# thu-ml/tianshou

Measured on AMD Instinct MI355X. Metric: PPO learn() update-steps/sec (minibatch 65536, preprocessing incl.) + GAE transitions/sec; cpu_baseline / rocm_eager_baseline are PORTS of the reference path (oracle/), kind=port, higher is better.
Workload: dtype f32; 1 GPU; C2 PPO MuJoCo-shape rollout (BASELINE configs[1]): ONE rollout of 512 envs x 2048 steps = 2^20 transitions, minibatch 65536, obs 17, act 6, MLP[64,64] actor-critic, repeat 10, recompute_advantage off; parallelism=dp1, exchange=none

## Files before the change

include/tsengine.h:

```cpp
#ifndef TSENGINE_H
#define TSENGINE_H

#include <stddef.h>
#include <stdint.h>

#ifdef __cplusplus
extern "C" {
#endif

#define TS_OK 0
#define TS_ERR_INVALID_ARG (-1)
#define TS_ERR_SHAPE (-2)
#define TS_ERR_HIP (-3)
#define TS_ERR_UNSUPPORTED (-4)
#define TS_ERR_WORKSPACE (-5)

typedef void* ts_stream_t;
typedef struct ts_workspace ts_workspace;

const char* ts_version(void);
const char* ts_last_error(void);

int ts_workspace_create(ts_workspace** out, int device, size_t max_bytes);
int ts_workspace_destroy(ts_workspace* ws);

int ts_workspace_side_stream(ts_workspace* ws, int which, ts_stream_t* stream_out);

#define TS_KIND_PPO_STEP 0
#define TS_KIND_PPO_REDUCE 1
#define TS_KIND_PPO_ADAM 2
#define TS_KIND_PPO_INFER 3
#define TS_KIND_GAE_MAPS 4
#define TS_KIND_GAE_APPLY 5
#define TS_KIND_CONV_FWD 6
#define TS_KIND_CONV_WGRAD 7
#define TS_KIND_CONV_DGRAD 8
#define TS_N_KINDS 9
int ts_profile_begin(ts_workspace* ws);
int ts_profile_end(ts_workspace* ws, double* h_ms_by_kind, int64_t* h_count_by_kind, int n_kinds);


int64_t ts_gae_num_tiles(int64_t n);
int ts_gae_scan(ts_workspace* ws, const float* v_s, const float* v_s_next, const void* rew,
                int rew_dtype, const uint8_t* terminated, const uint8_t* truncated,
                const int64_t* cut_pos, int64_t n_cut, const int64_t* d_n_cut, int64_t n,
                double gamma, double gae_lambda, double v_scale, double ret_div, float* adv_out,
                float* returns_out, double* adv64, double* ret64, double* ret_partials,
                ts_stream_t stream);

int ts_gae_check(ts_workspace* ws, int* h_error_out, ts_stream_t stream);

int ts_isin_positions(const int64_t* indices, int64_t n, const int64_t* unfinished,
                      int64_t n_unfinished, int64_t* cut_pos_out, int64_t capacity,
                      int64_t* n_cut_out, ts_stream_t stream);

int ts_nstep_return(const double* rew_B, const uint8_t* end_flag_B, const float* target_q_IA,
                    const int64_t* stacked_indices_NI, int64_t I, int64_t A, int64_t n_step,
                    int64_t B, double gamma, float* out, double* out64, ts_stream_t stream);

int ts_nstep_indices(const int64_t* indices, int64_t I, int64_t n_step, const int64_t* offset,
                     int64_t E, const uint8_t* done, const int64_t* last_index,
                     const int64_t* lengths, int64_t* after_out, int64_t* stacked_out,
                     ts_stream_t stream);

int ts_nstep_return_fused(const int64_t* indices, int64_t I, int64_t n_step,
                          const int64_t* offset, int64_t E, const uint8_t* done,
                          const uint8_t* terminated, const int64_t* last_index,
                          const int64_t* lengths, const double* rew_B, const float* target_q_IA,
                          int64_t A, double gamma, float* out, double* out64,
                          ts_stream_t stream);

int ts_nstep_coefficients(const int64_t* indices, int64_t I, int64_t n_step, const int64_t* offset, int64_t E,
                          const uint8_t* done_B, const uint8_t* terminated_B, const int64_t* last_index,
                          const int64_t* lengths, const double* rew_B, double gamma, float* mask_out, double* gpow_out,
                          double* mc_out, ts_stream_t stream);


int ts_next_index(const int64_t* index, int64_t I, const int64_t* offset, int64_t E,
                  const uint8_t* done, const int64_t* last_index, const int64_t* lengths,
                  int64_t* out, ts_stream_t stream);
int ts_prev_index(const int64_t* index, int64_t I, const int64_t* offset, int64_t E,
                  const uint8_t* done, const int64_t* last_index, const int64_t* lengths,
                  int64_t* out, ts_stream_t stream);

int ts_unfinished_index(const int64_t* offset, int64_t E, const uint8_t* done,
                        const int64_t* last_index, const int64_t* lengths, int64_t* out,
                        int64_t* n_out, ts_stream_t stream);

int ts_sample_indices_all(ts_workspace* ws, const int64_t* offset, int64_t E,
                          const int64_t* lengths, const int64_t* insertion, int64_t total,
                          int64_t* out, ts_stream_t stream);

int ts_sample_indices_random(const int64_t* offset, int64_t E, const int64_t* lengths, const double* u_buffer,
                             const int64_t* within_i, const double* within_u, int64_t batch_size, int64_t* out,
                             int* err_flag, ts_stream_t stream);
int ts_sample_indices_seeded(const int64_t* offset, int64_t E, const int64_t* lengths, uint64_t seed, uint64_t counter,
                             int64_t batch_size, int64_t* out, int* err_flag, ts_stream_t stream);

int ts_random_permutation(int64_t* out, int64_t n, uint64_t seed, ts_stream_t stream);

int ts_normal_fill(float* out, int64_t n, uint64_t seed, uint64_t offset, ts_stream_t stream);
// ... 728 lines not shown
```

tianshou_amd/csrc/ts_returns.hip:

```cpp
#include <algorithm>
#include <cstdlib>

#include "ts_common.h"

#pragma clang fp contract(off)

namespace {

constexpr int GAE_THREADS = 256;
constexpr int GAE_ITEMS = 8;
constexpr int GAE_TILE = GAE_THREADS * GAE_ITEMS;
constexpr int GAE_WAVES = GAE_THREADS / 64;

struct Aff {
    double a, b;
};

__device__ __forceinline__ Aff aff_identity() { return Aff{1.0, 0.0}; }

__device__ __forceinline__ Aff compose(const Aff& L, const Aff& R) {
    return Aff{L.a * R.a, L.b + L.a * R.b};
}

__device__ __forceinline__ Aff shfl_down_aff(const Aff& v, int off) {
    return Aff{__shfl_down(v.a, off, 64), __shfl_down(v.b, off, 64)};
}

__device__ __forceinline__ Aff wave_reduce_aff(Aff v, int lane) {
#pragma unroll
    for (int off = 1; off < 64; off <<= 1) {
        Aff r = shfl_down_aff(v, off);
        if (lane + off < 64) v = compose(v, r);
    }
    return v;
}

__device__ __forceinline__ Aff wave_suffix_scan_aff(Aff v, int lane) {
#pragma unroll
    for (int off = 1; off < 64; off <<= 1) {
        Aff r = shfl_down_aff(v, off);
        if (lane + off < 64) v = compose(v, r);
    }
    return v;
}

__device__ __forceinline__ Aff block_reduce_aff(Aff v, Aff* lds ) {
    const int lane = threadIdx.x & 63, wave = threadIdx.x >> 6;
    Aff w = wave_reduce_aff(v, lane);
    __syncthreads();
    if (lane == 0) lds[wave] = w;
    __syncthreads();
    Aff t = lds[0];
#pragma unroll
    for (int k = 1; k < GAE_WAVES; ++k) t = compose(t, lds[k]);
    return t;
}

template <typename RewT>
struct GaeArgs {
    const float* v_s;
    const float* v_n;
    const RewT* rew;
    const uint8_t* term;
    const uint8_t* trunc;
    const int64_t* cut_pos;
    const int64_t* d_n_cut;
    int64_t n_cut;
    int64_t n;
    double gamma, gl, v_scale, ret_div;
    const uint32_t* cutbits;
};

struct GaeRaw {
    float fv[GAE_ITEMS], fn[GAE_ITEMS];
    double rw[GAE_ITEMS];
    uint8_t te[GAE_ITEMS], tr[GAE_ITEMS];
};

template <typename RewT, bool VEC>
__device__ __forceinline__ void gae_load_raw(const GaeArgs<RewT>& g, int64_t base, GaeRaw& r) {
    const bool full = base + GAE_ITEMS <= g.n;
    if (VEC && full) {
        const float4* pv = reinterpret_cast<const float4*>(g.v_s + base);
        const float4* pn = reinterpret_cast<const float4*>(g.v_n + base);
        float4 a0 = pv[0], a1 = pv[1], b0 = pn[0], b1 = pn[1];
        r.fv[0] = a0.x; r.fv[1] = a0.y; r.fv[2] = a0.z; r.fv[3] = a0.w;
        r.fv[4] = a1.x; r.fv[5] = a1.y; r.fv[6] = a1.z; r.fv[7] = a1.w;
        r.fn[0] = b0.x; r.fn[1] = b0.y; r.fn[2] = b0.z; r.fn[3] = b0.w;
        r.fn[4] = b1.x; r.fn[5] = b1.y; r.fn[6] = b1.z; r.fn[7] = b1.w;
        if constexpr (sizeof(RewT) == 4) {
            const float4* pr = reinterpret_cast<const float4*>(g.rew + base);
            float4 r0 = pr[0], r1 = pr[1];
            r.rw[0] = r0.x; r.rw[1] = r0.y; r.rw[2] = r0.z; r.rw[3] = r0.w;
            r.rw[4] = r1.x; r.rw[5] = r1.y; r.rw[6] = r1.z; r.rw[7] = r1.w;
        } else {
            const double2* pr = reinterpret_cast<const double2*>(g.rew + base);
#pragma unroll
            for (int k = 0; k < GAE_ITEMS / 2; ++k) {
                double2 q = pr[k];
                r.rw[2 * k] = q.x;
                r.rw[2 * k + 1] = q.y;
            }
        }
        const uint2 t8 = *reinterpret_cast<const uint2*>(g.term + base);
        const uint2 u8 = *reinterpret_cast<const uint2*>(g.trunc + base);
#pragma unroll
        for (int k = 0; k < 4; ++k) {
            r.te[k] = (t8.x >> (8 * k)) & 0xFF;
            r.te[4 + k] = (t8.y >> (8 * k)) & 0xFF;
            r.tr[k] = (u8.x >> (8 * k)) & 0xFF;
            r.tr[4 + k] = (u8.y >> (8 * k)) & 0xFF;
        }
    } else {
#pragma unroll
        for (int k = 0; k < GAE_ITEMS; ++k) {
            const int64_t i = base + k;
            const bool ok = i < g.n;
            r.fv[k] = ok ? g.v_s[i] : 0.f;
            r.fn[k] = ok ? g.v_n[i] : 0.f;
            r.rw[k] = ok ? (double)g.rew[i] : 0.0;
            r.te[k] = ok ? g.term[i] : (uint8_t)1;
            r.tr[k] = ok ? g.trunc[i] : (uint8_t)1;
// ... 125 lines not shown
            if (base + k < g.n) {
                if (adv64) adv64[base + k] = adv[k];
                if (ret64) ret64[base + k] = ret[k];
            }
    }
}

__device__ __forceinline__ void gae_store_partials(double s1, double s2, int lane, int wave, int64_t tile,
                                                   double* red, double* ret_partials) {
#pragma unroll
    for (int off = 32; off > 0; off >>= 1) {
        s1 += __shfl_down(s1, off, 64);
        s2 += __shfl_down(s2, off, 64);
    }
    if (lane == 0) {
        red[2 * wave] = s1;
        red[2 * wave + 1] = s2;
    }
    __syncthreads();
    if (threadIdx.x == 0) {
        double t1 = 0.0, t2 = 0.0;
        for (int w = 0; w < GAE_WAVES; ++w) {
            t1 += red[2 * w];
            t2 += red[2 * w + 1];
        }
        ret_partials[2 * tile] = t1;
        ret_partials[2 * tile + 1] = t2;
    }
}

constexpr int GAE_SHARDS = 8;

struct GaeSyncHeader {
    struct alignas(128) { unsigned long long v; } ticket[GAE_SHARDS];
    unsigned int error;
    unsigned int pad[3];
};

struct GaeLaunch {
    unsigned long long base[GAE_SHARDS];
    int direct;
};

struct GaeTileMsg {
    unsigned long long a_bits, b_bits;
    unsigned int flag;
    unsigned int pad;
};

constexpr unsigned GAE_SPIN_LIMIT = 1u << 22;


template <typename RewT, bool VEC>
__global__ __launch_bounds__(GAE_THREADS) void gae_single_pass(GaeArgs<RewT> g, GaeSyncHeader* hdr,
                                                               GaeTileMsg* msg, int64_t n_tiles,
                                                               GaeLaunch launch,
                                                               unsigned int epoch, float* adv_out,
                                                               float* ret_out, double* adv64,
                                                               double* ret64, double* ret_partials) {
    __shared__ uint32_t cutmask[GAE_TILE / 32];
    __shared__ Aff lds[GAE_WAVES];
    __shared__ double red[2 * GAE_WAVES];
    __shared__ int64_t tile_s;
    __shared__ int closed_s;
    const int lane = threadIdx.x & 63, wave = threadIdx.x >> 6;
    int64_t tile;
    if (launch.direct) {
        tile = n_tiles - 1 - (int64_t)blockIdx.x;
    } else {
        if (threadIdx.x == 0) {
            const int shard = blockIdx.x & (GAE_SHARDS - 1);
            const unsigned long long t = __hip_atomic_fetch_add(&hdr->ticket[shard].v, 1ULL, __ATOMIC_RELAXED,
                                                                __HIP_MEMORY_SCOPE_AGENT);
            const int64_t seq = (int64_t)(t - launch.base[shard]) * GAE_SHARDS + shard;
            tile_s = n_tiles - 1 - seq;
        }
        __syncthreads();
        tile = tile_s;
    }
    const int64_t tile_start = tile * GAE_TILE;
    double vs[GAE_ITEMS], d[GAE_ITEMS], c[GAE_ITEMS];
    const int64_t base = tile_start + (int64_t)threadIdx.x * GAE_ITEMS;
    {
        GaeRaw raw;
        if (g.cutbits) {
            const GaeCutPre cuts = gae_cut_prefetch(g, tile_start);
            gae_load_raw<RewT, VEC>(g, base, raw);
            gae_cutmask_from_prefetch(g, tile_start, cuts, cutmask);
        } else {
            gae_load_raw<RewT, VEC>(g, base, raw);
            gae_build_cutmask(g, tile_start, cutmask);
        }
        gae_convert(g, base, raw, cutmask, vs, d, c);
    }
    const Aff mine = items_to_aff(d, c);

    const Aff incl = wave_suffix_scan_aff(mine, lane);
    Aff excl = shfl_down_aff(incl, 1);
    if (lane == 63) excl = aff_identity();
    if (lane == 0) lds[wave] = incl;
    if (threadIdx.x == GAE_THREADS - 1) closed_s = c[GAE_ITEMS - 1] == 0.0 ? 1 : 0;
    __syncthreads();
    const bool closed = closed_s != 0;
    Aff wmap[GAE_WAVES];
#pragma unroll
    for (int w = 0; w < GAE_WAVES; ++w) wmap[w] = lds[w];
    if (threadIdx.x == 0) {
        Aff t = wmap[0];
#pragma unroll
        for (int w = 1; w < GAE_WAVES; ++w) t = compose(t, wmap[w]);
        __hip_atomic_store(&msg[tile].a_bits, (unsigned long long)__double_as_longlong(t.a), __ATOMIC_RELAXED,
                           __HIP_MEMORY_SCOPE_AGENT);
        __hip_atomic_store(&msg[tile].b_bits, (unsigned long long)__double_as_longlong(t.b), __ATOMIC_RELAXED,
                           __HIP_MEMORY_SCOPE_AGENT);
        asm volatile("s_waitcnt vmcnt(0)" ::: "memory");
        __hip_atomic_store(&msg[tile].flag, epoch, __ATOMIC_RELAXED, __HIP_MEMORY_SCOPE_AGENT);
    }

    Aff acc = aff_identity();
    int64_t t0 = tile + 1;
    for (int round = 0; !closed && t0 < n_tiles; ++round) {
        const int width = round == 0 ? 1 : (round == 1 ? 15 : (round == 2 ? 240 : GAE_THREADS));
        Aff f = aff_identity();
        const int64_t t = t0 + threadIdx.x;
        if ((int)threadIdx.x < width && t < n_tiles) {
            unsigned spins = 0;
            while (__hip_atomic_load(&msg[t].flag, __ATOMIC_RELAXED, __HIP_MEMORY_SCOPE_AGENT) != epoch) {
                __builtin_amdgcn_s_sleep(1);
                if (++spins > GAE_SPIN_LIMIT) { hdr->error = 1u; break; }
            }
            const unsigned long long ab = __hip_atomic_load(&msg[t].a_bits, __ATOMIC_RELAXED, __HIP_MEMORY_SCOPE_AGENT);
            const unsigned long long bb = __hip_atomic_load(&msg[t].b_bits, __ATOMIC_RELAXED, __HIP_MEMORY_SCOPE_AGENT);
            f = Aff{__longlong_as_double((long long)ab), __longlong_as_double((long long)bb)};
        }
        acc = compose(acc, block_reduce_aff(f, lds));
        if (acc.a == 0.0) break;
        t0 += width;
    }
    double wave_carry = acc.b;
#pragma unroll
    for (int w = GAE_WAVES - 1; w >= 0; --w)
        if (w > wave) wave_carry = wmap[w].b + wmap[w].a * wave_carry;
    double x = excl.b + excl.a * wave_carry;

    double adv[GAE_ITEMS], ret[GAE_ITEMS];
    double s1 = 0.0, s2 = 0.0;
#pragma unroll
    for (int k = GAE_ITEMS - 1; k >= 0; --k) {
        x = d[k] + c[k] * x;
        adv[k] = x;
        ret[k] = x + vs[k];
        if (base + k < g.n) {
            s1 += ret[k];
            s2 += ret[k] * ret[k];
        }
    }
    gae_store_outputs<VEC>(g, base, adv, ret, adv_out, ret_out, adv64, ret64);
    if (ret_partials) gae_store_partials(s1, s2, lane, wave, tile, red, ret_partials);
}

__global__ void isin_positions_kernel(const int64_t* indices, int64_t n, const int64_t* unf,
                                      int64_t n_unf, int64_t* out, int64_t capacity,
                                      unsigned long long* count) {
    const int64_t stride = (int64_t)gridDim.x * blockDim.x;
    for (int64_t i = (int64_t)blockIdx.x * blockDim.x + threadIdx.x; i < n; i += stride) {
        const int64_t v = indices[i];
        int64_t lo = 0, hi = n_unf;
        while (lo < hi) {
            const int64_t mid = (lo + hi) >> 1;
            if (unf[mid] < v) lo = mid + 1; else hi = mid;
        }
        if (lo < n_unf && unf[lo] == v) {
            const unsigned long long p = atomicAdd(count, 1ULL);
            if ((int64_t)p < capacity) out[p] = i;
        }
    }
}

__device__ __forceinline__ int64_t pymod(int64_t a, int64_t m) {
    const int64_t r = a % m;
    return r < 0 ? r + m : r;
}

__device__ __forceinline__ int64_t find_sub(const int64_t* offset, int64_t E, int64_t idx) {
    int64_t lo = 0, hi = E;
    while (hi - lo > 1) {
        const int64_t mid = (lo + hi) >> 1;
        if (offset[mid] <= idx) lo = mid; else hi = mid;
    }
    return lo;
}

__device__ __forceinline__ int64_t next_one(int64_t idx, const int64_t* offset, int64_t E,
                                            const uint8_t* done, const int64_t* last_index,
                                            const int64_t* lengths, bool* is_end) {
    idx = pymod(idx, offset[E]);
    const int64_t e = find_sub(offset, E, idx);
    const int64_t start = offset[e];
    const int64_t len = lengths[e];
    const int64_t cur_len = len > 1 ? len : 1;
    const int64_t end_flag = (done[idx] != 0) | (idx == last_index[e]);
    if (is_end) *is_end = (done[idx] != 0) | (len > 0 && idx == last_index[e]);
    return pymod(idx - start + 1 - end_flag, cur_len) + start;
}

__global__ void nstep_return_kernel(const double* rew, const uint8_t* end_flag, const float* tq,
                                    const int64_t* stacked, int64_t I, int64_t A, int64_t N,
                                    double gamma, float* out, double* out64) {
    const int64_t total = I * A;
    const int64_t stride = (int64_t)gridDim.x * blockDim.x;
    for (int64_t t = (int64_t)blockIdx.x * blockDim.x + threadIdx.x; t < total; t += stride) {
// ... 155 lines not shown
int launch_gae(ts_workspace* ws, const GaeArgs<RewT>& g_in, float* adv_out, float* ret_out,
               double* adv64, double* ret64, double* ret_partials, hipStream_t stream) {
    GaeArgs<RewT> g = g_in;
    const int64_t n_tiles = ts::ceil_div(g.n, GAE_TILE);
    g.cutbits = nullptr;
    if (g.n_cut > GAE_CUT_SCAN_MAX) {
        const size_t words = (size_t)ts::ceil_div(g.n, 32);
        if (int rc = ts::ws_reserve(ws, 4 * words)) return rc;
        uint32_t* bits = reinterpret_cast<uint32_t*>(ws->base);
        TS_HIP_CHECK(hipMemsetAsync(bits, 0, 4 * words, stream));
        const unsigned blocks = (unsigned)std::min<int64_t>(ts::ceil_div(g.n_cut, 256), 1024);
        hipLaunchKernelGGL(gae_cutbits_kernel, dim3(blocks), dim3(256), 0, stream, g.cut_pos, g.n_cut, g.d_n_cut, g.n, bits);
        TS_LAUNCH_CHECK();
        g.cutbits = bits;
    }
    const bool vec = aligned16(g.v_s) && aligned16(g.v_n) && aligned16(g.rew) &&
                     (reinterpret_cast<uintptr_t>(g.term) & 7u) == 0 &&
                     (reinterpret_cast<uintptr_t>(g.trunc) & 7u) == 0 && aligned16(adv_out) &&
                     aligned16(ret_out);
    {
        int rc = gae_sync_reserve(ws, n_tiles, stream);
        if (rc != TS_OK) return rc;
        GaeSyncHeader* hdr = reinterpret_cast<GaeSyncHeader*>(ws->gae_sync);
        GaeTileMsg* msg = reinterpret_cast<GaeTileMsg*>(hdr + 1);
        const unsigned int epoch = ++ws->gae_epoch;
        GaeLaunch base;
        static const int64_t direct_max = getenv("TS_GAE_DIRECT_MAX") ? atoll(getenv("TS_GAE_DIRECT_MAX")) : 1024;
        base.direct = n_tiles <= direct_max ? 1 : 0;
        for (int k = 0; k < GAE_SHARDS; ++k) {
            base.base[k] = ws->gae_ticket_base[k];
            if (!base.direct)
                ws->gae_ticket_base[k] += (unsigned long long)((n_tiles - k + GAE_SHARDS - 1) / GAE_SHARDS);
        }
        ts::ProfScope prof(ws, TS_KIND_GAE_APPLY, stream);
        if (vec)
            hipLaunchKernelGGL((gae_single_pass<RewT, true>), dim3((unsigned)n_tiles), dim3(GAE_THREADS), 0,
                               stream, g, hdr, msg, n_tiles, base, epoch, adv_out, ret_out, adv64, ret64,
                               ret_partials);
        else
            hipLaunchKernelGGL((gae_single_pass<RewT, false>), dim3((unsigned)n_tiles), dim3(GAE_THREADS), 0,
                               stream, g, hdr, msg, n_tiles, base, epoch, adv_out, ret_out, adv64, ret64,
                               ret_partials);
        TS_LAUNCH_CHECK();
        return TS_OK;
    }
}

}

extern "C" {

int64_t ts_gae_num_tiles(int64_t n) { return n <= 0 ? 0 : ts::ceil_div(n, GAE_TILE); }

int ts_gae_scan(ts_workspace* ws, const float* v_s, const float* v_s_next, const void* rew,
                int rew_dtype, const uint8_t* terminated, const uint8_t* truncated,
                const int64_t* cut_pos, int64_t n_cut, const int64_t* d_n_cut, int64_t n,
                double gamma, double gae_lambda, double v_scale, double ret_div, float* adv_out,
                float* returns_out, double* adv64, double* ret64, double* ret_partials,
                ts_stream_t stream) {
    TS_REQUIRE(n >= 0 && n_cut >= 0, TS_ERR_INVALID_ARG, "ts_gae_scan: negative size");
    if (n == 0) return TS_OK;
    TS_REQUIRE(v_s && v_s_next && rew && terminated && truncated && adv_out && returns_out,
               TS_ERR_INVALID_ARG, "ts_gae_scan: NULL array argument");
    TS_REQUIRE(n_cut == 0 || cut_pos, TS_ERR_INVALID_ARG, "ts_gae_scan: cut_pos is NULL");
    TS_REQUIRE(rew_dtype == 0 || rew_dtype == 1, TS_ERR_INVALID_ARG,
               "ts_gae_scan: rew_dtype must be 0 (f32) or 1 (f64)");
    TS_REQUIRE(ret_div != 0.0, TS_ERR_INVALID_ARG, "ts_gae_scan: ret_div must be non-zero");
    hipStream_t s = ts::as_stream(stream);
    if (rew_dtype == 0) {
        GaeArgs<float> g{v_s, v_s_next, (const float*)rew, terminated, truncated, cut_pos, d_n_cut,
                         n_cut, n, gamma, gamma * gae_lambda, v_scale, ret_div};
        return launch_gae(ws, g, adv_out, returns_out, adv64, ret64, ret_partials, s);
    }
    GaeArgs<double> g{v_s, v_s_next, (const double*)rew, terminated, truncated, cut_pos, d_n_cut,
                      n_cut, n, gamma, gamma * gae_lambda, v_scale, ret_div};
    return launch_gae(ws, g, adv_out, returns_out, adv64, ret64, ret_partials, s);
}

int ts_gae_check(ts_workspace* ws, int* error_out, ts_stream_t stream) {
    TS_REQUIRE(ws && error_out, TS_ERR_INVALID_ARG, "ts_gae_check: NULL argument");
    *error_out = 0;
    if (!ws->gae_sync) return TS_OK;
    GaeSyncHeader h;
    hipStream_t s = ts::as_stream(stream);
    TS_HIP_CHECK(hipMemcpyAsync(&h, ws->gae_sync, sizeof(h), hipMemcpyDeviceToHost, s));
    TS_HIP_CHECK(hipStreamSynchronize(s));
    *error_out = (int)h.error;
    return TS_OK;
}

int ts_isin_positions(const int64_t* indices, int64_t n, const int64_t* unfinished,
                      int64_t n_unfinished, int64_t* cut_pos_out, int64_t capacity,
                      int64_t* n_cut_out, ts_stream_t stream) {
    TS_REQUIRE(n >= 0 && n_unfinished >= 0 && capacity >= 0, TS_ERR_INVALID_ARG,
               "ts_isin_positions: negative size");
    TS_REQUIRE(n_cut_out, TS_ERR_INVALID_ARG, "ts_isin_positions: n_cut_out is NULL");
    hipStream_t s = ts::as_stream(stream);
    TS_HIP_CHECK(hipMemsetAsync(n_cut_out, 0, sizeof(int64_t), s));
    if (n == 0 || n_unfinished == 0) return TS_OK;
    TS_REQUIRE(indices && unfinished && cut_pos_out, TS_ERR_INVALID_ARG,
               "ts_isin_positions: NULL array argument");
    hipLaunchKernelGGL(isin_positions_kernel, dim3(grid_for(n, 256)), dim3(256), 0, s, indices, n,
                       unfinished, n_unfinished, cut_pos_out, capacity,
                       reinterpret_cast<unsigned long long*>(n_cut_out));
    TS_LAUNCH_CHECK();
    return TS_OK;
}

int ts_nstep_return(const double* rew_B, const uint8_t* end_flag_B, const float* target_q_IA,
                    const int64_t* stacked_indices_NI, int64_t I, int64_t A, int64_t n_step,
                    int64_t B, double gamma, float* out, double* out64, ts_stream_t stream) {
    TS_REQUIRE(I >= 0 && A >= 0 && B >= 0, TS_ERR_INVALID_ARG, "ts_nstep_return: negative size");
    TS_REQUIRE(n_step >= 1, TS_ERR_INVALID_ARG, "ts_nstep_return: n_step must be >= 1");
    if (I * A == 0) return TS_OK;
    TS_REQUIRE(rew_B && end_flag_B && target_q_IA && stacked_indices_NI && out, TS_ERR_INVALID_ARG,
               "ts_nstep_return: NULL array argument");
    hipLaunchKernelGGL(nstep_return_kernel, dim3(grid_for(I * A, 256)), dim3(256), 0,
                       ts::as_stream(stream), rew_B, end_flag_B, target_q_IA, stacked_indices_NI, I,
                       A, n_step, gamma, out, out64);
    TS_LAUNCH_CHECK();
    return TS_OK;
}

int ts_nstep_indices(const int64_t* indices, int64_t I, int64_t n_step, const int64_t* offset,
                     int64_t E, const uint8_t* done, const int64_t* last_index,
                     const int64_t* lengths, int64_t* after_out, int64_t* stacked_out,
                     ts_stream_t stream) {
    TS_REQUIRE(I >= 0 && E >= 1, TS_ERR_INVALID_ARG, "ts_nstep_indices: bad size");
    TS_REQUIRE(n_step >= 1, TS_ERR_INVALID_ARG, "ts_nstep_indices: n_step must be >= 1");
// ... 50 lines not shown
```

tianshou_amd/ppo.py:

```python
from __future__ import annotations

import ctypes as C
import math
from dataclasses import dataclass

import numpy as np
import torch

from . import _lib
from .buffer import _dev_index
from .returns import gae_scan

HIDDEN = 64
PARAM_ORDER = ("a_w1", "a_b1", "a_w2", "a_b2", "a_wmu", "a_bmu", "a_sigma",
               "c_w1", "c_b1", "c_w2", "c_b2", "c_wv", "c_bv")


def param_shapes(obs_dim: int, act_dim: int) -> dict[str, tuple[int, ...]]:
    return {
        "a_w1": (HIDDEN, obs_dim), "a_b1": (HIDDEN,), "a_w2": (HIDDEN, HIDDEN), "a_b2": (HIDDEN,),
        "a_wmu": (act_dim, HIDDEN), "a_bmu": (act_dim,), "a_sigma": (act_dim,),
        "c_w1": (HIDDEN, obs_dim), "c_b1": (HIDDEN,), "c_w2": (HIDDEN, HIDDEN), "c_b2": (HIDDEN,),
        "c_wv": (1, HIDDEN), "c_bv": (1,),
    }


def param_count(obs_dim: int, act_dim: int) -> int:
    return int(_lib.load().ts_ppo_param_count(_lib.i64(obs_dim), _lib.i64(act_dim)))


TIANSHOU_ACTOR_KEYS = ("preprocess.model.model.0.weight", "preprocess.model.model.0.bias",
                       "preprocess.model.model.2.weight", "preprocess.model.model.2.bias",
                       "mu.model.0.weight", "mu.model.0.bias", "sigma_param")
TIANSHOU_CRITIC_KEYS = ("preprocess.model.model.0.weight", "preprocess.model.model.0.bias",
                        "preprocess.model.model.2.weight", "preprocess.model.model.2.bias",
                        "last.model.0.weight", "last.model.0.bias")


def flat_from_modules(actor, critic, device="cuda") -> torch.Tensor:
    sa, sc = actor.state_dict(), critic.state_dict()
    parts = [sa[k] for k in TIANSHOU_ACTOR_KEYS] + [sc[k] for k in TIANSHOU_CRITIC_KEYS]
    return torch.cat([p.detach().reshape(-1).to(torch.float32) for p in parts]).to(device).contiguous()


def flat_to_modules(flat: torch.Tensor, actor, critic) -> None:
    off = 0
    with torch.no_grad():
        for mod, keys in ((actor, TIANSHOU_ACTOR_KEYS), (critic, TIANSHOU_CRITIC_KEYS)):
            sd = dict(mod.named_parameters())
            for k in keys:
                p = sd[k]
                n = p.numel()
                p.copy_(flat[off:off + n].reshape(p.shape).to(p.device))
                off += n
    assert off == flat.numel()


@dataclass
class PPOConfig:
    algo: str = "ppo"
    gamma: float = 0.99
    gae_lambda: float = 0.95
    eps_clip: float = 0.2
    dual_clip: float | None = None
# ... 69 lines not shown
    ws = _lib.default_workspace(_dev_index(params))
    _lib.check(_lib.load().ts_ppo_infer_bounded(
        ws.handle, _lib.ptr(params), _lib.i64(obs_dim), _lib.i64(act_dim), _lib.f64(max_action or 0.0), _lib.ptr(obs),
        _lib.ptr(act), _lib.i64(n), _lib.ptr(v), _lib.ptr(lp), None, _lib.current_stream(dev)))
    return v, lp


def policy_forward(params: torch.Tensor, obs_dim: int, act_dim: int, obs: torch.Tensor, noise=None, *,
                   bound_method: str | None = "clip", low=None, high=None, max_action: float | None = None,
                   want_mu: bool = False):
    n, dev = obs.shape[0], obs.device
    obs = obs.to(torch.float32).contiguous()
    noise = None if noise is None else torch.as_tensor(noise, device=dev).to(torch.float32).reshape(n, act_dim).contiguous()
    f = lambda x: None if x is None else torch.as_tensor(x, dtype=torch.float32, device=dev).reshape(act_dim).contiguous()
    low, high = f(low), f(high)
    act = torch.empty((n, act_dim), dtype=torch.float32, device=dev)
    mapped = torch.empty_like(act)
    mu = torch.empty_like(act) if want_mu else None
    ws = _lib.default_workspace(_dev_index(params))
    _lib.check(_lib.load().ts_ppo_policy_forward_bounded(
        ws.handle, _lib.ptr(params), _lib.i64(obs_dim), _lib.i64(act_dim), _lib.f64(max_action or 0.0), _lib.ptr(obs),
        _lib.ptr(noise), _lib.i64(n), C.c_int({None: 0, "clip": 1, "tanh": 2}[bound_method]), _lib.ptr(low), _lib.ptr(high),
        _lib.ptr(act), _lib.ptr(mapped), _lib.ptr(mu), _lib.current_stream(dev)))
    return (act, mapped, mu) if want_mu else (act, mapped)


def pack_batch(b: dict, obs_dim: int, act_dim: int) -> torch.Tensor:
    n = b["obs"].shape[0]
    lib = _lib.load()
    lib.ts_ppo_record_width.restype = C.c_int64
    w = int(lib.ts_ppo_record_width(_lib.i64(obs_dim), _lib.i64(act_dim)))
    rec = torch.empty((n, w), dtype=torch.float32, device=b["obs"].device)
    _lib.check(lib.ts_ppo_pack_batch(
        _lib.ptr(b["obs"]), _lib.ptr(b["act"]), _lib.ptr(b["adv"]), _lib.ptr(b["returns"]),
        _lib.ptr(b["logp_old"]), _lib.ptr(b["v_s"]), _lib.i64(n), _lib.i64(obs_dim), _lib.i64(act_dim),
        _lib.ptr(rec), _lib.current_stream(rec.device)))
    return rec


class PPOEngine:

    def __init__(self, obs_dim: int, act_dim: int, flat_params: torch.Tensor, cfg: PPOConfig):
        if not flat_params.is_cuda:
            raise RuntimeError("PPOEngine needs its parameters on an MI355X; there is no CPU fallback")
        self.obs_dim, self.act_dim, self.cfg = obs_dim, act_dim, cfg
        self.P = param_count(obs_dim, act_dim)
        if flat_params.numel() != self.P:
            raise ValueError(f"flat_params has {flat_params.numel()} entries, layout needs {self.P}")
        self.params = flat_params.detach().to(torch.float32).contiguous().clone()
        self.adam_m = torch.zeros_like(self.params)
        self.adam_v = torch.zeros_like(self.params)
        self.adam_step = 0
        self.device = self.params.device
        self.ret_rms = [0.0, 1.0, 0.0]
        self._eps = 1e-8
        self._ws = _lib.default_workspace(_dev_index(self.params))

    def check(self) -> None:
        if self._ws.gae_check():
            raise _lib.EngineError(-1, "gae_single_pass: a tile hand-off timed out; advantages / returns are invalid")

    def _f32(self, x) -> torch.Tensor:
        if not isinstance(x, torch.Tensor):
            x = torch.as_tensor(np.asarray(x), device=self.device)
        return x.to(device=self.device, dtype=torch.float32).contiguous()

    def add_returns_and_advantages(self, obs, obs_next, rew, terminated, truncated, cut_pos,
                                   d_n_cut=None, reduce_stats=None, v_s=None):
        cfg = self.cfg
        if v_s is None:
            v_s, _ = infer(self.params, self.obs_dim, self.act_dim, obs)
        v_next, _ = infer(self.params, self.obs_dim, self.act_dim, obs_next)
        scale = math.sqrt(self.ret_rms[1] + self._eps) if cfg.return_scaling else 1.0
        out = gae_scan(v_s, v_next, rew, terminated, truncated, cut_pos, gamma=cfg.gamma,
                       gae_lambda=cfg.gae_lambda, v_scale=scale, ret_div=scale,
                       want_ret_stats=cfg.return_scaling, d_n_cut=d_n_cut, ws=self._ws)
        if cfg.return_scaling:
            n = float(v_s.numel())
            s1, s2 = float(out["ret_sum"]), float(out["ret_sumsq"])
            if reduce_stats is not None:
                s1, s2, n = reduce_stats(s1, s2, n)
            self.ret_rms = rms_merge(self.ret_rms, s1, s2, n)
        return v_s, out["returns"], out["adv"]

    def preprocess(self, obs, obs_next, act, rew, terminated, truncated, cut_pos, d_n_cut=None, reduce_stats=None):
        obs, obs_next, act = self._f32(obs), self._f32(obs_next), self._f32(act)
        if self.cfg.algo == "a2c":
            v_s, returns, adv = self.add_returns_and_advantages(obs, obs_next, rew, terminated,
                                                                truncated, cut_pos, d_n_cut, reduce_stats)
            logp_old = torch.zeros_like(adv)
        else:
            v_s0, logp_old = infer(self.params, self.obs_dim, self.act_dim, obs, act, want_v=True, want_logp=True,
                                   max_action=self.cfg.max_action)
            v_s, returns, adv = self.add_returns_and_advantages(obs, obs_next, rew, terminated, truncated, cut_pos,
                                                                d_n_cut, reduce_stats, v_s=v_s0)
        return {"obs": obs, "obs_next": obs_next, "act": act, "rew": rew, "terminated": terminated,
                "truncated": truncated, "cut_pos": cut_pos, "d_n_cut": d_n_cut,
                "v_s": v_s, "returns": returns, "adv": adv, "logp_old": logp_old}

    def _run_steps(self, b: dict, perm: torch.Tensor | None, offsets: list[int], want_grad=False):
        n_steps = len(offsets) - 1
        losses = torch.empty((n_steps, 4), dtype=torch.float32, device=self.device)
        grads = torch.empty(self.P, dtype=torch.float32, device=self.device) if want_grad else None
        h_off = (C.c_int64 * len(offsets))(*offsets)
        hp = self.cfg.to_c()
        _lib.check(_lib.load().ts_ppo_update(
            self._ws.handle, _lib.ptr(self.params), _lib.ptr(self.adam_m), _lib.ptr(self.adam_v),
            _lib.i64(self.adam_step), _lib.i64(self.obs_dim), _lib.i64(self.act_dim),
            _lib.ptr(b["obs"]), _lib.ptr(b["act"]), _lib.ptr(b["adv"]), _lib.ptr(b["returns"]),
            _lib.ptr(b["logp_old"]), _lib.ptr(b["v_s"]), _lib.i64(b["obs"].shape[0]), _lib.ptr(perm),
            h_off, _lib.i64(n_steps), C.byref(hp), _lib.ptr(losses), _lib.ptr(grads),
            _lib.current_stream(self.device)))
        self.adam_step += n_steps
        return losses, grads

    def update(self, b: dict, batch_size: int | None, repeat: int, perms=None, want_grad=False):
        n = b["obs"].shape[0]
        cfg = self.cfg
        if perms is None:
            perms = [np.random.permutation(n) for _ in range(repeat)]
        offs1 = split_offsets(n, batch_size, merge_last=True)
        out, grads = [], None
        if not cfg.recompute_advantage:
            if all(isinstance(p, torch.Tensor) for p in perms):
                perm = torch.cat([p.to(device=self.device, dtype=torch.int64) for p in perms])
            else:
                perm = torch.as_tensor(np.concatenate([np.asarray(p, dtype=np.int64) for p in perms]),
                                       device=self.device)
            offsets = [r * n + o for r in range(repeat) for o in offs1[:-1]] + [repeat * n]
            losses, grads = self._run_steps(b, perm, offsets, want_grad)
            out.append(losses)
        else:
            for r in range(repeat):
                if r > 0:
                    v_s, returns, adv = self.add_returns_and_advantages(
# ... 17 lines not shown
```

tianshou_amd/returns.py:

```python
from __future__ import annotations

import numpy as np
import torch

from . import _lib
from .buffer import DeviceReplayBuffer, _dev_index, _i64_dev, _u8_dev


def _f32(x, device) -> torch.Tensor:
    if isinstance(x, torch.Tensor):
        return x.to(device=device, dtype=torch.float32).reshape(-1).contiguous()
    return torch.as_tensor(np.asarray(x, dtype=np.float32).reshape(-1), device=device)


def gae_scan(v_s, v_s_next, rew, terminated, truncated, cut_pos=None, *, gamma=0.99,
             gae_lambda=0.95, v_scale=1.0, ret_div=1.0, want_f64=False, want_ret_stats=False,
             d_n_cut=None, ws=None):
    dev = v_s.device
    v_s = _f32(v_s, dev)
    v_s_next = _f32(v_s_next, dev)
    n = v_s.numel()
    if isinstance(rew, torch.Tensor):
        rew = rew.to(dev).reshape(-1)
        if rew.dtype not in (torch.float32, torch.float64):
            rew = rew.to(torch.float64)
        rew = rew.contiguous()
    else:
        rew = torch.as_tensor(np.asarray(rew, dtype=np.float64).reshape(-1), device=dev)
    terminated, truncated = _u8_dev(terminated, dev).reshape(-1), _u8_dev(truncated, dev).reshape(-1)
    if not (v_s_next.numel() == rew.numel() == terminated.numel() == truncated.numel() == n):
        raise ValueError("gae_scan: input length mismatch")
    n_cut = 0
    if cut_pos is not None:
        cut_pos = _i64_dev(cut_pos, dev).reshape(-1)
        n_cut = cut_pos.numel()
    adv = torch.empty(n, dtype=torch.float32, device=dev)
    ret = torch.empty(n, dtype=torch.float32, device=dev)
    adv64 = torch.empty(n, dtype=torch.float64, device=dev) if want_f64 else None
    ret64 = torch.empty(n, dtype=torch.float64, device=dev) if want_f64 else None
    lib = _lib.load()
    parts = None
    if want_ret_stats:
        parts = torch.zeros(2 * max(int(lib.ts_gae_num_tiles(n)), 1), dtype=torch.float64, device=dev)
    if ws is None:
        ws = _lib.default_workspace(_dev_index(v_s))
    _lib.check(lib.ts_gae_scan(
        ws.handle, _lib.ptr(v_s), _lib.ptr(v_s_next), _lib.ptr(rew),
        0 if rew.dtype == torch.float32 else 1, _lib.ptr(terminated), _lib.ptr(truncated),
        _lib.ptr(cut_pos), _lib.i64(n_cut), _lib.ptr(d_n_cut), _lib.i64(n), _lib.f64(gamma),
        _lib.f64(gae_lambda), _lib.f64(v_scale), _lib.f64(ret_div), _lib.ptr(adv), _lib.ptr(ret),
        _lib.ptr(adv64), _lib.ptr(ret64), _lib.ptr(parts), _lib.current_stream(dev)))
    out = {"adv": adv, "returns": ret}
    if want_f64:
        out["adv64"], out["ret64"] = adv64, ret64
    if want_ret_stats:
        p = parts.view(-1, 2).sum(dim=0)
        out["ret_sum"], out["ret_sumsq"] = p[0], p[1]
    return out


def _gae(v_s, v_s_, rew, end_flag, gamma: float, gae_lambda: float) -> torch.Tensor:
    dev = v_s.device if isinstance(v_s, torch.Tensor) else torch.device("cuda")
    end = _u8_dev(end_flag, dev)
    zeros = torch.zeros_like(end)
    return gae_scan(_f32(v_s, dev), _f32(v_s_, dev), rew, zeros, end, gamma=gamma,
                    gae_lambda=gae_lambda, want_f64=True)["adv64"]


def cut_positions(buffer: DeviceReplayBuffer, indices: torch.Tensor):
    dev = buffer.device
    unf, n_unf = buffer._unfinished_raw()
    indices = _i64_dev(indices, dev).reshape(-1)
    pad = torch.full_like(unf, torch.iinfo(torch.int64).max)
    ar = torch.arange(unf.numel(), device=dev)
    unf_sorted = torch.where(ar < n_unf, unf, pad)
    cut = torch.empty(max(unf.numel(), 1), dtype=torch.int64, device=dev)
    d_n = torch.zeros(1, dtype=torch.int64, device=dev)
    _lib.check(_lib.load().ts_isin_positions(
        _lib.ptr(indices), _lib.i64(indices.numel()), _lib.ptr(unf_sorted), _lib.i64(unf.numel()),
        _lib.ptr(cut), _lib.i64(cut.numel()), _lib.ptr(d_n), _lib.current_stream(dev)))
    return cut, d_n


def compute_episodic_return(batch, buffer: DeviceReplayBuffer, indices, v_s_=None, v_s=None,
                            gamma: float = 0.99, gae_lambda: float = 0.95):
    dev = buffer.device
    rew = batch.rew
    n = rew.numel()
    if v_s_ is None:
        if not np.isclose(gae_lambda, 1.0):
            raise AssertionError("v_s_ is None requires gae_lambda == 1.0")
        v_next = torch.zeros(n, dtype=torch.float32, device=dev)
    else:
        v_next = _f32(v_s_, dev)
    term = _u8_dev(batch.terminated, dev).reshape(-1)
    if v_s is None:
        v_cur = torch.roll(v_next * (term == 0).to(torch.float32), 1)
    else:
        v_cur = _f32(v_s, dev)
    cut, d_n = cut_positions(buffer, indices)
    out = gae_scan(v_cur, v_next, rew, term, batch.truncated, cut, gamma=gamma,
                   gae_lambda=gae_lambda, want_f64=True, d_n_cut=d_n)
    return out["ret64"], out["adv64"]


def _nstep_return(rew_B, end_flag_B, target_q_IA, stacked_indices_NI, gamma: float,
                  n_step: int, want_f64: bool = False):
    dev = target_q_IA.device
    tq = target_q_IA.to(torch.float32).contiguous()
    I = tq.shape[0]
    A = tq.numel() // max(I, 1)
# ... 81 lines not shown
```

Baseline: 16430 update-steps/s.

## Keep return-RMS state on device to remove host sync in PPO preprocessing

Moves the running return mean/variance update from host Python to a single-thread device kernel, and has the GAE kernel read its scale from a device pointer. This removes the blocking float() reads of the return sums after the GAE scan, which stalled the host each learn() call. The host copy is fetched lazily only when ret_rms is read. It adds a tiny kernel launch and a pinned H2D copy when the state is reset, and keeps an env var escape hatch to the old host path.

```diff
diff --git a/include/tsengine.h b/include/tsengine.h
--- a/include/tsengine.h
+++ b/include/tsengine.h
@@ -47,6 +47,15 @@
                 double gamma, double gae_lambda, double v_scale, double ret_div, float* adv_out,
                 float* returns_out, double* adv64, double* ret64, double* ret_partials,
                 ts_stream_t stream);
+
+int ts_gae_scan_dev(ts_workspace* ws, const float* v_s, const float* v_s_next, const void* rew,
+                    int rew_dtype, const uint8_t* terminated, const uint8_t* truncated,
+                    const int64_t* cut_pos, int64_t n_cut, const int64_t* d_n_cut, int64_t n,
+                    double gamma, double gae_lambda, const double* scale_dev, float* adv_out,
+                    float* returns_out, double* adv64, double* ret64, double* ret_partials,
+                    ts_stream_t stream);
+
+int ts_ret_rms_merge(ts_workspace* ws, const double* sums, int64_t n, double* state, double eps, ts_stream_t stream);
 
 int ts_gae_check(ts_workspace* ws, int* h_error_out, ts_stream_t stream);
 
diff --git a/tianshou_amd/csrc/ts_ret_rms.h b/tianshou_amd/csrc/ts_ret_rms.h
--- /dev/null
+++ b/tianshou_amd/csrc/ts_ret_rms.h
@@ -0,0 +1,54 @@
+#pragma once
+#include <cmath>
+#include <cstdint>
+#include <cstring>
+
+#if defined(__HIPCC__)
+#define TS_HD __host__ __device__
+#else
+#define TS_HD
+#endif
+
+namespace ts {
+
+TS_HD inline double f64_step(double y, int64_t by) {
+    int64_t b;
+    memcpy(&b, &y, 8);
+    b += by;
+    memcpy(&y, &b, 8);
+    return y;
+}
+
+TS_HD inline double sqrt_fixup(double x, double y) {
+#if defined(__clang__)
+#pragma clang fp contract(off)
+#endif
+    if (!(x >= 2.2250738585072014e-308) || !(x <= 1.7976931348623157e308)) return y;
+    const double up = f64_step(y, 1), dn = f64_step(y, -1);
+    const double r = fma(-y, y, x);
+    if (r > y * (up - y)) return up;
+    if (r <= -(y * (y - dn))) return dn;
+    return y;
+}
+
+TS_HD inline double sqrt_rn(double x) { return sqrt_fixup(x, sqrt(x)); }
+
+TS_HD inline void ret_rms_merge(double* state, double s1, double s2, double n, double eps) {
+#if defined(__clang__)
+#pragma clang fp contract(off)
+#endif
+    const double b_mean = s1 / n;
+    const double raw = s2 / n - b_mean * b_mean;
+    const double b_var = 0.0 > raw ? 0.0 : raw;
+    const double mean = state[0], var = state[1], count = state[2];
+    const double delta = b_mean - mean;
+    const double tot = count + n;
+    const double m2 = var * count + b_var * n + delta * delta * count * n / tot;
+    const double var_new = m2 / tot;
+    state[0] = mean + delta * n / tot;
+    state[1] = var_new;
+    state[2] = tot;
+    state[3] = sqrt_rn(var_new + eps);
+}
+
+}
diff --git a/tianshou_amd/csrc/ts_returns.hip b/tianshou_amd/csrc/ts_returns.hip
--- a/tianshou_amd/csrc/ts_returns.hip
+++ b/tianshou_amd/csrc/ts_returns.hip
@@ -2,6 +2,7 @@
 #include <cstdlib>
 
 #include "ts_common.h"
+#include "ts_ret_rms.h"
 
 #pragma clang fp contract(off)
 
@@ -68,6 +69,7 @@
     int64_t n_cut;
     int64_t n;
     double gamma, gl, v_scale, ret_div;
+    const double* scale_dev;
     const uint32_t* cutbits;
 };
 
@@ -299,7 +301,7 @@
 
 
 template <typename RewT, bool VEC>
-__global__ __launch_bounds__(GAE_THREADS) void gae_single_pass(GaeArgs<RewT> g, GaeSyncHeader* hdr,
+__global__ __launch_bounds__(GAE_THREADS) void gae_single_pass(GaeArgs<RewT> g_in, GaeSyncHeader* hdr,
                                                                GaeTileMsg* msg, int64_t n_tiles,
                                                                GaeLaunch launch,
                                                                unsigned int epoch, float* adv_out,
@@ -311,6 +313,12 @@
     __shared__ int64_t tile_s;
     __shared__ int closed_s;
     const int lane = threadIdx.x & 63, wave = threadIdx.x >> 6;
+    GaeArgs<RewT> g = g_in;
+    if (g.scale_dev) {
+        const double scale = *g.scale_dev;
+        g.v_scale = scale;
+        g.ret_div = scale;
+    }
     int64_t tile;
     if (launch.direct) {
         tile = n_tiles - 1 - (int64_t)blockIdx.x;
@@ -404,6 +412,10 @@
     }
     gae_store_outputs<VEC>(g, base, adv, ret, adv_out, ret_out, adv64, ret64);
     if (ret_partials) gae_store_partials(s1, s2, lane, wave, tile, red, ret_partials);
+}
+
+__global__ void ret_rms_merge_kernel(const double* __restrict__ sums, double n, double* __restrict__ state, double eps) {
+    if (blockIdx.x == 0 && threadIdx.x == 0) ts::ret_rms_merge(state, sums[0], sums[1], n, eps);
 }
 
 __global__ void isin_positions_kernel(const int64_t* indices, int64_t n, const int64_t* unf,
@@ -665,12 +677,12 @@
 
 int64_t ts_gae_num_tiles(int64_t n) { return n <= 0 ? 0 : ts::ceil_div(n, GAE_TILE); }
 
-int ts_gae_scan(ts_workspace* ws, const float* v_s, const float* v_s_next, const void* rew,
-                int rew_dtype, const uint8_t* terminated, const uint8_t* truncated,
-                const int64_t* cut_pos, int64_t n_cut, const int64_t* d_n_cut, int64_t n,
-                double gamma, double gae_lambda, double v_scale, double ret_div, float* adv_out,
-                float* returns_out, double* adv64, double* ret64, double* ret_partials,
-                ts_stream_t stream) {
+static int gae_scan_impl(ts_workspace* ws, const float* v_s, const float* v_s_next, const void* rew,
+                         int rew_dtype, const uint8_t* terminated, const uint8_t* truncated,
+                         const int64_t* cut_pos, int64_t n_cut, const int64_t* d_n_cut, int64_t n,
+                         double gamma, double gae_lambda, double v_scale, double ret_div, const double* scale_dev,
+                         float* adv_out, float* returns_out, double* adv64, double* ret64, double* ret_partials,
+                         ts_stream_t stream) {
     TS_REQUIRE(n >= 0 && n_cut >= 0, TS_ERR_INVALID_ARG, "ts_gae_scan: negative size");
     if (n == 0) return TS_OK;
     TS_REQUIRE(v_s && v_s_next && rew && terminated && truncated && adv_out && returns_out,
@@ -682,12 +694,42 @@
     hipStream_t s = ts::as_stream(stream);
     if (rew_dtype == 0) {
         GaeArgs<float> g{v_s, v_s_next, (const float*)rew, terminated, truncated, cut_pos, d_n_cut,
-                         n_cut, n, gamma, gamma * gae_lambda, v_scale, ret_div};
+                         n_cut, n, gamma, gamma * gae_lambda, v_scale, ret_div, scale_dev};
         return launch_gae(ws, g, adv_out, returns_out, adv64, ret64, ret_partials, s);
     }
     GaeArgs<double> g{v_s, v_s_next, (const double*)rew, terminated, truncated, cut_pos, d_n_cut,
-                      n_cut, n, gamma, gamma * gae_lambda, v_scale, ret_div};
+                      n_cut, n, gamma, gamma * gae_lambda, v_scale, ret_div, scale_dev};
     return launch_gae(ws, g, adv_out, returns_out, adv64, ret64, ret_partials, s);
+}
+
+int ts_gae_scan(ts_workspace* ws, const float* v_s, const float* v_s_next, const void* rew,
+                int rew_dtype, const uint8_t* terminated, const uint8_t* truncated,
+                const int64_t* cut_pos, int64_t n_cut, const int64_t* d_n_cut, int64_t n,
+                double gamma, double gae_lambda, double v_scale, double ret_div, float* adv_out,
+                float* returns_out, double* adv64, double* ret64, double* ret_partials,
+                ts_stream_t stream) {
+    return gae_scan_impl(ws, v_s, v_s_next, rew, rew_dtype, terminated, truncated, cut_pos, n_cut, d_n_cut, n, gamma,
+                         gae_lambda, v_scale, ret_div, nullptr, adv_out, returns_out, adv64, ret64, ret_partials, stream);
+}
+
+int ts_gae_scan_dev(ts_workspace* ws, const float* v_s, const float* v_s_next, const void* rew,
+                    int rew_dtype, const uint8_t* terminated, const uint8_t* truncated,
+                    const int64_t* cut_pos, int64_t n_cut, const int64_t* d_n_cut, int64_t n,
+                    double gamma, double gae_lambda, const double* scale_dev, float* adv_out,
+                    float* returns_out, double* adv64, double* ret64, double* ret_partials,
+                    ts_stream_t stream) {
+    TS_REQUIRE(scale_dev, TS_ERR_INVALID_ARG, "ts_gae_scan_dev: scale_dev is NULL");
+    return gae_scan_impl(ws, v_s, v_s_next, rew, rew_dtype, terminated, truncated, cut_pos, n_cut, d_n_cut, n, gamma,
+                         gae_lambda, 1.0, 1.0, scale_dev, adv_out, returns_out, adv64, ret64, ret_partials, stream);
+}
+
+int ts_ret_rms_merge(ts_workspace* ws, const double* sums, int64_t n, double* state, double eps, ts_stream_t stream) {
+    (void)ws;
+    TS_REQUIRE(sums && state, TS_ERR_INVALID_ARG, "ts_ret_rms_merge: NULL argument");
+    TS_REQUIRE(n >= 1, TS_ERR_INVALID_ARG, "ts_ret_rms_merge: the batch needs at least one return");
+    hipLaunchKernelGGL(ret_rms_merge_kernel, dim3(1), dim3(1), 0, ts::as_stream(stream), sums, (double)n, state, eps);
+    TS_LAUNCH_CHECK();
+    return TS_OK;
 }
 
 int ts_gae_check(ts_workspace* ws, int* error_out, ts_stream_t stream) {
diff --git a/tianshou_amd/ppo.py b/tianshou_amd/ppo.py
--- a/tianshou_amd/ppo.py
+++ b/tianshou_amd/ppo.py
@@ -2,6 +2,7 @@
 
 import ctypes as C
 import math
+import os
 from dataclasses import dataclass
 
 import numpy as np
@@ -9,7 +10,7 @@
 
 from . import _lib
 from .buffer import _dev_index
-from .returns import gae_scan
+from .returns import gae_scan, ret_rms_merge
 
 HIDDEN = 64
 PARAM_ORDER = ("a_w1", "a_b1", "a_w2", "a_b2", "a_wmu", "a_bmu", "a_sigma",
@@ -185,9 +186,28 @@
         self.adam_v = torch.zeros_like(self.params)
         self.adam_step = 0
         self.device = self.params.device
-        self.ret_rms = [0.0, 1.0, 0.0]
         self._eps = 1e-8
         self._ws = _lib.default_workspace(_dev_index(self.params))
+        self._rms_host, self._rms_dev = None, None
+        self.ret_rms = [0.0, 1.0, 0.0]
+
+    @property
+    def ret_rms(self) -> list:
+        if self._rms_host is None:
+            self._rms_host = self._rms_dev[:3].tolist()
+        return list(self._rms_host)
+
+    @ret_rms.setter
+    def ret_rms(self, value) -> None:
+        mean, var, count = (float(x) for x in value)
+        self._rms_host, self._rms_dev = [mean, var, count], None
+
+    def _rms_state(self) -> torch.Tensor:
+        if self._rms_dev is None:
+            mean, var, count = self._rms_host
+            host = torch.tensor([mean, var, count, math.sqrt(var + self._eps)], dtype=torch.float64).pin_memory()
+            self._rms_dev = host.to(self.device, non_blocking=True)
+        return self._rms_dev
 
     def check(self) -> None:
         if self._ws.gae_check():
@@ -204,7 +224,16 @@
         if v_s is None:
             v_s, _ = infer(self.params, self.obs_dim, self.act_dim, obs)
         v_next, _ = infer(self.params, self.obs_dim, self.act_dim, obs_next)
-        scale = math.sqrt(self.ret_rms[1] + self._eps) if cfg.return_scaling else 1.0
+        if cfg.return_scaling and reduce_stats is None and os.environ.get("TS_PPO_HOST_RMS") != "1":
+            state = self._rms_state()
+            out = gae_scan(v_s, v_next, rew, terminated, truncated, cut_pos, gamma=cfg.gamma,
+                           gae_lambda=cfg.gae_lambda, scale_dev=state[3:], want_ret_stats=True, d_n_cut=d_n_cut,
+                           ws=self._ws)
+            ret_rms_merge(state, out["ret_sums"], v_s.numel(), self._eps, ws=self._ws)
+            self._rms_host = None
+            return v_s, out["returns"], out["adv"]
+        rms = self.ret_rms
+        scale = math.sqrt(rms[1] + self._eps) if cfg.return_scaling else 1.0
         out = gae_scan(v_s, v_next, rew, terminated, truncated, cut_pos, gamma=cfg.gamma,
                        gae_lambda=cfg.gae_lambda, v_scale=scale, ret_div=scale,
                        want_ret_stats=cfg.return_scaling, d_n_cut=d_n_cut, ws=self._ws)
@@ -213,7 +242,7 @@
             s1, s2 = float(out["ret_sum"]), float(out["ret_sumsq"])
             if reduce_stats is not None:
                 s1, s2, n = reduce_stats(s1, s2, n)
-            self.ret_rms = rms_merge(self.ret_rms, s1, s2, n)
+            self.ret_rms = rms_merge(rms, s1, s2, n)
         return v_s, out["returns"], out["adv"]
 
     def preprocess(self, obs, obs_next, act, rew, terminated, truncated, cut_pos, d_n_cut=None, reduce_stats=None):
diff --git a/tianshou_amd/returns.py b/tianshou_amd/returns.py
--- a/tianshou_amd/returns.py
+++ b/tianshou_amd/returns.py
@@ -15,7 +15,7 @@
 
 def gae_scan(v_s, v_s_next, rew, terminated, truncated, cut_pos=None, *, gamma=0.99,
              gae_lambda=0.95, v_scale=1.0, ret_div=1.0, want_f64=False, want_ret_stats=False,
-             d_n_cut=None, ws=None):
+             d_n_cut=None, ws=None, scale_dev=None):
     dev = v_s.device
     v_s = _f32(v_s, dev)
     v_s_next = _f32(v_s_next, dev)
@@ -44,19 +44,39 @@
         parts = torch.zeros(2 * max(int(lib.ts_gae_num_tiles(n)), 1), dtype=torch.float64, device=dev)
     if ws is None:
         ws = _lib.default_workspace(_dev_index(v_s))
-    _lib.check(lib.ts_gae_scan(
-        ws.handle, _lib.ptr(v_s), _lib.ptr(v_s_next), _lib.ptr(rew),
-        0 if rew.dtype == torch.float32 else 1, _lib.ptr(terminated), _lib.ptr(truncated),
-        _lib.ptr(cut_pos), _lib.i64(n_cut), _lib.ptr(d_n_cut), _lib.i64(n), _lib.f64(gamma),
-        _lib.f64(gae_lambda), _lib.f64(v_scale), _lib.f64(ret_div), _lib.ptr(adv), _lib.ptr(ret),
-        _lib.ptr(adv64), _lib.ptr(ret64), _lib.ptr(parts), _lib.current_stream(dev)))
+    if scale_dev is None:
+        _lib.check(lib.ts_gae_scan(
+            ws.handle, _lib.ptr(v_s), _lib.ptr(v_s_next), _lib.ptr(rew),
+            0 if rew.dtype == torch.float32 else 1, _lib.ptr(terminated), _lib.ptr(truncated),
+            _lib.ptr(cut_pos), _lib.i64(n_cut), _lib.ptr(d_n_cut), _lib.i64(n), _lib.f64(gamma),
+            _lib.f64(gae_lambda), _lib.f64(v_scale), _lib.f64(ret_div), _lib.ptr(adv), _lib.ptr(ret),
+            _lib.ptr(adv64), _lib.ptr(ret64), _lib.ptr(parts), _lib.current_stream(dev)))
+    else:
+        if scale_dev.dtype != torch.float64 or scale_dev.device != dev or scale_dev.numel() < 1:
+            raise ValueError("gae_scan: scale_dev must be a float64 tensor on the inputs' device")
+        _lib.check(lib.ts_gae_scan_dev(
+            ws.handle, _lib.ptr(v_s), _lib.ptr(v_s_next), _lib.ptr(rew),
+            0 if rew.dtype == torch.float32 else 1, _lib.ptr(terminated), _lib.ptr(truncated),
+            _lib.ptr(cut_pos), _lib.i64(n_cut), _lib.ptr(d_n_cut), _lib.i64(n), _lib.f64(gamma),
+            _lib.f64(gae_lambda), _lib.ptr(scale_dev), _lib.ptr(adv), _lib.ptr(ret),
+            _lib.ptr(adv64), _lib.ptr(ret64), _lib.ptr(parts), _lib.current_stream(dev)))
     out = {"adv": adv, "returns": ret}
     if want_f64:
         out["adv64"], out["ret64"] = adv64, ret64
     if want_ret_stats:
         p = parts.view(-1, 2).sum(dim=0)
-        out["ret_sum"], out["ret_sumsq"] = p[0], p[1]
+        out["ret_sum"], out["ret_sumsq"], out["ret_sums"] = p[0], p[1], p
     return out
+
+
+def ret_rms_merge(state: torch.Tensor, sums: torch.Tensor, n: int, eps: float = 1e-8, ws=None) -> None:
+    for t, k in ((state, 4), (sums, 2)):
+        if t.dtype != torch.float64 or t.numel() != k:
+            raise ValueError("ret_rms_merge: state is float64[4], sums is float64[2]")
+    if ws is None:
+        ws = _lib.default_workspace(_dev_index(state))
+    _lib.check(_lib.load().ts_ret_rms_merge(ws.handle, _lib.ptr(sums), _lib.i64(n), _lib.ptr(state), _lib.f64(eps),
+                                            _lib.current_stream(state.device)))
 
 
 def _gae(v_s, v_s_, rew, end_flag, gamma: float, gae_lambda: float) -> torch.Tensor:
```

Result: no change. 16420 update-steps/s (-0.1%).
